# continental/uncertainty-detection-autolabeling

Measured on AMD Instinct MI355X. Metric: images*MC-samples/sec, EfficientDet-D0 MC-dropout serve (preprocess+net xT+decode+NMS), higher is better.
Workload: dtype f32 (tensors and accumulators float32; 1x1 products on the matrix cores as two fp16 pieces per operand, 3 cross terms (~2^-22 per product; float32-class, the default))

## Files before the change

uncertainty-detection-autolabeling_amd/csrc/kernels_pwb.hip:

```cpp
#include <math.h>
#include <stdio.h>
#include <stdlib.h>
#include <string.h>

#include <type_traits>

#include "mfma_common.h"

namespace uda {

template <int MT, int NT, int WM, int WN, int PARTS, int OCC, bool DEEP = false>
__global__ __launch_bounds__(256, OCC) void pwb_kernel(PwArgs a) {
  static_assert(WM * WN == 4, "four waves per block");
  constexpr int NPC = split_np(PARTS);
  constexpr int BM = 32 * MT * WM, NTB = NT * WN, BN = 32 * NTB;
  constexpr int A_BYTES = NPC * BM * PWB_AROW;
  constexpr int B_BYTES = 2 * NTB * NPC * 1024;
  constexpr int STG_BYTES = 4 * 32 * PWB_STG * 4;
  constexpr int LDS_BYTES = (A_BYTES + B_BYTES) > STG_BYTES ? (A_BYTES + B_BYTES) : STG_BYTES;
  __shared__ __attribute__((aligned(16))) unsigned char lds[LDS_BYTES];
  unsigned char* As = lds;
  uint4* Bs = (uint4*)(lds + A_BYTES);

  const int tid = threadIdx.x, lane = tid & 63, wave = tid >> 6;
// ... 265 lines not shown
#pragma unroll
    for (int p = 0; p < 2; ++p)
      bf[ks][p] = __builtin_bit_cast(bf16x8, ks < KS ? Wp[(((size_t)ks * NTL) * 2 + p) * 64 + lane] : make_uint4(0u, 0u, 0u, 0u));
  const int rrow = lane >> 4, c4 = lane & 15;
  const int col = 4 * c4;
  const bool colok = col < a.Cout;
  float4 bias = make_float4(0.f, 0.f, 0.f, 0.f), sc = make_float4(1.f, 1.f, 1.f, 1.f), sh = make_float4(0.f, 0.f, 0.f, 0.f);
  if (colok && (a.Cout & 3) == 0) {
    if (a.bias) bias = *(const float4*)(a.bias + col);
    if (a.bn_scale) { sc = *(const float4*)(a.bn_scale + col); sh = *(const float4*)(a.bn_shift + col); }
  }

  for (int t = 0; t < a.in_div; ++t) {
    const int b = b_in * a.in_div + t;
    float4 rg = make_float4(1.f, 1.f, 1.f, 1.f);
    if (a.se) {
      const int k = 4 * (lane & 7);
      if (k < a.Cin) rg = *(const float4*)(a.se + (size_t)(b / a.se_div) * a.Cin + k);
    }
#pragma unroll
    for (int i = 0; i < 4; ++i) {
      const int m = (lane >> 3) + 8 * i, kq = lane & 7;
      float r0 = ra[i].x * rg.x, r1 = ra[i].y * rg.y, r2 = ra[i].z * rg.z, r3 = ra[i].w * rg.w;
#pragma unroll
      for (int p = 0; p < 2; ++p) {
        const unsigned u0 = pack_bf16(r0, r1), u1 = pack_bf16(r2, r3);
        *(uint2*)(Aw + (size_t)(p * 32 + m) * PWB_AROW + kq * 8) = make_uint2(u0, u1);
        if (p == 0) {
          r0 -= bf16_lo_f32(u0); r1 -= bf16_hi_f32(u0);
          r2 -= bf16_lo_f32(u1); r3 -= bf16_hi_f32(u1);
        }
      }
    }
    __builtin_amdgcn_wave_barrier();
    f32x16 acc;
#pragma unroll
    for (int r = 0; r < 16; ++r) acc[r] = 0.f;
#pragma unroll
    for (int ks = 0; ks < 2; ++ks) {
      const bf16x8 a0 = *(const bf16x8*)(Aw + (size_t)(0 * 32 + li) * PWB_AROW + ks * 32 + lh * 16);
      const bf16x8 a1 = *(const bf16x8*)(Aw + (size_t)(1 * 32 + li) * PWB_AROW + ks * 32 + lh * 16);
      acc = __builtin_amdgcn_mfma_f32_32x32x16_bf16(a1, bf[ks][0], acc, 0, 0, 0);
      acc = __builtin_amdgcn_mfma_f32_32x32x16_bf16(a0, bf[ks][1], acc, 0, 0, 0);
      acc = __builtin_amdgcn_mfma_f32_32x32x16_bf16(a0, bf[ks][0], acc, 0, 0, 0);
    }
    __builtin_amdgcn_wave_barrier();
#pragma unroll
    for (int r = 0; r < 16; ++r) stg[((r & 3) + 8 * (r >> 2) + 4 * lh) * PWB_STG + li] = acc[r];
    __builtin_amdgcn_wave_barrier();
    float4 mk = make_float4(1.f, 1.f, 1.f, 1.f);
    if (colok && a.mask) mk = *(const float4*)(a.mask + (size_t)b * a.Cout + col);
    const size_t out_base = (size_t)b * a.HW;
    const size_t res_base = a.res ? (size_t)(b / a.res_div) * a.HW : 0;
#pragma unroll
    for (int it = 0; it < 8; ++it) {
      const int row = it * 4 + rrow;
      const int m = m0 + row;
      if (colok && m < a.HW) {
        float4 v = *(const float4*)(stg + row * PWB_STG + col);
        v.x = fmaf(v.x + bias.x, sc.x, sh.x);
        v.y = fmaf(v.y + bias.y, sc.y, sh.y);
        v.z = fmaf(v.z + bias.z, sc.z, sh.z);
        v.w = fmaf(v.w + bias.w, sc.w, sh.w);
        if (a.act == UDA_ACT_SWISH) {
          v.x = swishf_b(v.x); v.y = swishf_b(v.y); v.z = swishf_b(v.z); v.w = swishf_b(v.w);
        } else if (a.act >= UDA_ACT_RELU) {
          v.x = act_relu_family(v.x, a.act); v.y = act_relu_family(v.y, a.act); v.z = act_relu_family(v.z, a.act); v.w = act_relu_family(v.w, a.act);
        }
        v.x *= mk.x; v.y *= mk.y; v.z *= mk.z; v.w *= mk.w;
        if (a.res) {
          const float4 rr = *(const float4*)(a.res + (res_base + m) * a.Cout + col);
          v.x += rr.x; v.y += rr.y; v.z += rr.z; v.w += rr.w;
        }
        *(float4*)(a.out + (out_base + m) * a.Cout + col) = v;
      }
    }
    __builtin_amdgcn_wave_barrier();
  }
}

#ifndef UDA_PWS_D
#define UDA_PWS_D 4
#endif
constexpr int PWS_D = UDA_PWS_D;
template <int PARTS, int NT, bool GATE, bool IH = false>
__global__ __launch_bounds__(64) void pws_kernel(PwArgs a) {
  constexpr int NPC = split_np(PARTS);
  const int lane = threadIdx.x, li = lane & 31, lh = lane >> 5;
  const int m0 = blockIdx.x * 32, nt0 = blockIdx.y * NT;
  const int b = blockIdx.z, b_in = b / a.in_div;
  const int KS = a.Cin >> 4;
  const int NTL = (a.Cout + 31) >> 5;
  const int mr = m0 + li < a.HW ? m0 + li : a.HW - 1;
  const float* arow = a.in + ((size_t)b_in * a.HW + mr) * a.Cin + 8 * lh;
  constexpr bool in_h = IH;
  const unsigned short* arow_h = (const unsigned short*)a.in + ((size_t)b_in * a.HW + mr) * a.Cin + 8 * lh;
  const float* se = GATE ? a.se + (size_t)(b / a.se_div) * a.Cin + 8 * lh : nullptr;
  const uint4* Wp = (const uint4*)a.wsplit + lane;
  size_t woff[NT];
#pragma unroll
  for (int n = 0; n < NT; ++n) woff[n] = (size_t)(nt0 + n < NTL ? nt0 + n : NTL - 1) * NPC * 64;
  const size_t wks = (size_t)NTL * NPC * 64;

  f32x16 acc[NT];
#pragma unroll
  for (int n = 0; n < NT; ++n)
#pragma unroll
    for (int r = 0; r < 16; ++r) acc[n][r] = 0.f;
  float amax = 0.f;

  struct Step { float4 a0, a1, g0, g1; uint4 w[NT][NPC]; };
  struct Group { Step s[PWS_D]; };
  auto load_step = [&](int ks, Step& t) {
    if constexpr (in_h) {
      const uint4 h = *(const uint4*)(arow_h + 16 * ks);
      t.a0 = make_float4(__uint_as_float(h.x), __uint_as_float(h.y), __uint_as_float(h.z), __uint_as_float(h.w));
      t.a1 = t.a0;
    } else {
      t.a0 = *(const float4*)(arow + 16 * ks);
      t.a1 = *(const float4*)(arow + 16 * ks + 4);
    }
    if constexpr (GATE) {
      t.g0 = *(const float4*)(se + 16 * ks);
      t.g1 = *(const float4*)(se + 16 * ks + 4);
    }
#pragma unroll
    for (int n = 0; n < NT; ++n)
#pragma unroll
      for (int p = 0; p < NPC; ++p) t.w[n][p] = Wp[(size_t)ks * wks + woff[n] + p * 64];
  };
  auto mma_step = [&](const Step& t) {
    float4 v0 = t.a0, v1 = t.a1;
    if constexpr (in_h) {
      v0 = half4_to_float4<PARTS>(__float_as_uint(t.a0.x), __float_as_uint(t.a0.y));
      v1 = half4_to_float4<PARTS>(__float_as_uint(t.a0.z), __float_as_uint(t.a0.w));
    }
    if constexpr (GATE) {
      v0.x *= t.g0.x; v0.y *= t.g0.y; v0.z *= t.g0.z; v0.w *= t.g0.w;
      v1.x *= t.g1.x; v1.y *= t.g1.y; v1.z *= t.g1.z; v1.w *= t.g1.w;
    }
    bf16x8 af[NPC];
    split_parts<PARTS>(v0, v1, af, amax);
#pragma unroll
    for (int n = 0; n < NT; ++n) {
      bf16x8 bf[NPC];
#pragma unroll
      for (int p = 0; p < NPC; ++p) bf[p] = __builtin_bit_cast(bf16x8, t.w[n][p]);
      acc[n] = mfma_terms<PARTS>(af, bf, acc[n]);
    }
  };
  auto load_group = [&](int g, Group& G) {
#pragma unroll
    for (int d = 0; d < PWS_D; ++d) load_step(g * PWS_D + d, G.s[d]);
  };
  auto mma_group = [&](const Group& G) {
#pragma unroll
    for (int d = 0; d < PWS_D; ++d) mma_step(G.s[d]);
  };
  const int ng = KS / PWS_D;
  Group c0, c1;
  load_group(0, c0);
  load_group(ng > 1 ? 1 : 0, c1);
#pragma unroll 1
  for (int g = 0; g < ng; g += 2) {
    mma_group(c0);
    load_group(g + 2 < ng ? g + 2 : ng - 1, c0);
    if (g + 1 < ng) mma_group(c1);
    load_group(g + 3 < ng ? g + 3 : ng - 1, c1);
  }
#pragma unroll 1
  for (int ks = ng * PWS_D; ks < KS; ++ks) {
    Step t;
    load_step(ks, t);
    mma_step(t);
  }
  split_report<PARTS>(amax, a.oor);

  const size_t out_base = (size_t)b * a.HW;
  const float un = a.wunscale;
  const size_t res_base = a.res ? (size_t)(b / a.res_div) * a.HW : 0;
#pragma unroll
  for (int n = 0; n < NT; ++n) {
    const int col = (nt0 + n) * 32 + li;
    if (nt0 + n >= NTL || col >= a.Cout) continue;
    const float bias = a.bias ? a.bias[col] : 0.f;
    const float sc = a.bn_scale ? a.bn_scale[col] : 1.f;
    const float sh = a.bn_scale ? a.bn_shift[col] : 0.f;
    const float mk = a.mask ? a.mask[(size_t)b * a.Cout + col] : 1.f;
#pragma unroll
    for (int r = 0; r < 16; ++r) {
      const int m = m0 + (r & 3) + 8 * (r >> 2) + 4 * lh;
      if (m >= a.HW) continue;
      float v = fmaf(acc[n][r], un, bias);
      v = fmaf(v, sc, sh);
      if (a.act == UDA_ACT_SWISH) v = swishf_b(v);
      else if (a.act >= UDA_ACT_RELU) v = act_relu_family(v, a.act);
      v *= mk;
      if (a.res) v += a.res[(res_base + m) * a.Cout + col];
      a.out[(out_base + m) * a.Cout + col] = v;
    }
  }
}

static int launch_pws(const PwArgs& a, int rows, hipStream_t s) {
  static long long max_work = -1;
  if (max_work < 0) { const char* e = getenv("UDA_PW_SKINNY"); max_work = e ? atoll(e) : 60000; }
  if ((long long)rows * a.HW * ((a.Cout + 31) / 32) > max_work || a.Cin < 256 || (a.Cin & 15) || !a.wsplit || a.wparts == UDA_SPLIT_NONE) return 0;
  const int row_tiles = (a.HW + 31) / 32, NTL = (a.Cout + 31) / 32;
  const int nt = ((long long)row_tiles * rows * NTL <= 1024) ? 1 : 2;
  const dim3 grid(row_tiles, (NTL + nt - 1) / nt, rows), block(64);
  auto go = [&](auto k1, auto k2) { if (nt == 1) hipLaunchKernelGGL(k1, grid, block, 0, s, a); else hipLaunchKernelGGL(k2, grid, block, 0, s, a); };
  if (a.wparts == UDA_SPLIT_F16X2) { if (a.se) go(pws_kernel<4, 1, true>, pws_kernel<4, 2, true>); else go(pws_kernel<4, 1, false>, pws_kernel<4, 2, false>); }
  else if (a.wparts == UDA_SPLIT_F16X1 && a.in_f16) { if (a.se) go(pws_kernel<5, 1, true, true>, pws_kernel<5, 2, true, true>); else go(pws_kernel<5, 1, false, true>, pws_kernel<5, 2, false, true>); }
  else if (a.wparts == UDA_SPLIT_F16X1) { if (a.se) go(pws_kernel<5, 1, true>, pws_kernel<5, 2, true>); else go(pws_kernel<5, 1, false>, pws_kernel<5, 2, false>); }
  else if (a.wparts == UDA_SPLIT_BF16X1 && a.in_f16) { if (a.se) go(pws_kernel<6, 1, true, true>, pws_kernel<6, 2, true, true>); else go(pws_kernel<6, 1, false, true>, pws_kernel<6, 2, false, true>); }
  else if (a.wparts == UDA_SPLIT_BF16X1) { if (a.se) go(pws_kernel<6, 1, true>, pws_kernel<6, 2, true>); else go(pws_kernel<6, 1, false>, pws_kernel<6, 2, false>); }
  else if (a.wparts == UDA_SPLIT_BF16X3) { if (a.se) go(pws_kernel<3, 1, true>, pws_kernel<3, 2, true>); else go(pws_kernel<3, 1, false>, pws_kernel<3, 2, false>); }
  else if (a.wparts == UDA_SPLIT_BF16X2) { if (a.se) go(pws_kernel<2, 1, true>, pws_kernel<2, 2, true>); else go(pws_kernel<2, 1, false>, pws_kernel<2, 2, false>); }
  else return 0;
  return 1;
}

template <int MT, int NT, int WM, int WN>
static void launch_pwb_cfg(const PwArgs& a, int rows, hipStream_t s) {
  constexpr int BM = 32 * MT * WM, BN = 32 * NT * WN;
  const dim3 grid((a.HW + BM - 1) / BM, (a.Cout + BN - 1) / BN, rows), block(256);
  if (a.wparts == UDA_SPLIT_BF16X3) hipLaunchKernelGGL((pwb_kernel<MT, NT, WM, WN, 3, 2>), grid, block, 0, s, a);
  else if (a.wparts == UDA_SPLIT_F16X1) {
    hipLaunchKernelGGL((pwb_kernel<MT, NT, WM, WN, 5, (MT * NT > 5 ? 2 : 3)>), grid, block, 0, s, a);
  }
  else if (a.wparts == UDA_SPLIT_BF16X1) hipLaunchKernelGGL((pwb_kernel<MT, NT, WM, WN, 6, (MT * NT > 5 ? 2 : 3)>), grid, block, 0, s, a);
  else if (a.wparts == UDA_SPLIT_F16X2) {
    if constexpr (MT * NT > 4) {
      if (a.Cin >= 384 && a.Cin % PWB_BK == 0 && a.Cout % BN == 0 && (2 * NT * WN * 2 * 64) % 256 == 0) { hipLaunchKernelGGL((pwb_kernel<MT, NT, WM, WN, 4, 2, true>), grid, block, 0, s, a); return; }
    }
    hipLaunchKernelGGL((pwb_kernel<MT, NT, WM, WN, 4, (MT * NT > 4 ? 2 : 3)>), grid, block, 0, s, a);
  }
  else hipLaunchKernelGGL((pwb_kernel<MT, NT, WM, WN, 2, (MT * NT > 4 ? 2 : 3)>), grid, block, 0, s, a);
}

void launch_pwb(const PwArgs& a, int rows, hipStream_t s) {
  static const int shared = uda_env_int("UDA_PW_SHARED", 1);
  if (shared && a.in_div > 1 && a.Cin <= 32 && a.Cout <= 32 && (a.Cout & 3) == 0 && a.wparts == 2 && rows % a.in_div == 0) {
    const dim3 grid((a.HW + 127) / 128, 1, rows / a.in_div);
    hipLaunchKernelGGL(pwb_shared_kernel, grid, dim3(256), 0, s, a);
    return;
  }
  if (launch_pws(a, rows, s)) return;
  int cfg = a.Cout <= 32 ? 1 : (a.Cout <= 64 ? 2 : (a.Cout <= 96 ? 3 : 4));
  if (a.Cout > 128) {
    const int bn[3] = {128, 160, 192}, id[3] = {4, 6, 5};
    int best = 1 << 30;
    for (int i = 0; i < 3; ++i) {
      const int waste = (a.Cout + bn[i] - 1) / bn[i] * bn[i] - a.Cout;
      if (waste <= best) { best = waste; cfg = id[i]; }
    }
  }
  switch (cfg) {
    case 1: launch_pwb_cfg<1, 1, 4, 1>(a, rows, s); break;
    case 2: launch_pwb_cfg<1, 2, 4, 1>(a, rows, s); break;
    case 3: launch_pwb_cfg<1, 3, 4, 1>(a, rows, s); break;
    case 5: launch_pwb_cfg<2, 3, 2, 2>(a, rows, s); break;
    case 6: launch_pwb_cfg<1, 5, 4, 1>(a, rows, s); break;
    default: launch_pwb_cfg<2, 2, 2, 2>(a, rows, s); break;
  }
}

#ifndef UDA_MBX_ET
#define UDA_MBX_ET 3
#endif
__host__ __device__ constexpr int mbx_et_w(int k, int s) {
  return s != 1 ? 0 : (k == 5 ? ((UDA_MBX_ET & 1) ? 4 : 0) : ((UDA_MBX_ET & 2) ? 2 : 0));
}
__host__ __device__ constexpr int mbx_et_pitch(int w) { return w == 2 ? 258 : 260; }
template <int W>
__device__ __forceinline__ void et_store_slice(float* ep, const f32x16& acc) {
#pragma unroll
  for (int q = 0; q < 4; ++q) {
    const float v0 = swish_core(acc[4 * q]), v1 = swish_core(acc[4 * q + 1]), v2 = swish_core(acc[4 * q + 2]), v3 = swish_core(acc[4 * q + 3]);
    if constexpr (W == 4) {
      *(float4*)(ep + 8 * q) = make_float4(v0, v1, v2, v3);
    } else {
      *(float2*)(ep + 8 * q) = make_float2(v0, v1);
      *(float2*)(ep + 8 * q + 2) = make_float2(v2, v3);
    }
  }
}
template <int W>
__device__ __forceinline__ void et_read(float* dst, const float* er, int jj) {
  if constexpr (W == 4) {
    const float4 v = *(const float4*)(er + 4 * jj);
    dst[4 * jj] = v.x; dst[4 * jj + 1] = v.y; dst[4 * jj + 2] = v.z; dst[4 * jj + 3] = v.w;
  } else {
    const float2 v = *(const float2*)(er + 2 * jj);
    dst[2 * jj] = v.x; dst[2 * jj + 1] = v.y;
  }
}

namespace {
struct MbxCfgB { int th, tw; };
__host__ __device__ constexpr MbxCfgB mbxb_cfg(int k, int s) {
  return s == 1 ? (k == 3 ? MbxCfgB{12, 16} : MbxCfgB{8, 16}) : (k == 3 ? MbxCfgB{7, 8} : MbxCfgB{4, 10});
}
}

#ifndef UDA_MBXB_WK_LDS
#define UDA_MBXB_WK_LDS 1
#endif
#ifndef UDA_MBXB6_W
#define UDA_MBXB6_W 3
#endif
#ifndef UDA_MBXB_MINW
#define UDA_MBXB_MINW(K, S, KSF, PARTS) ((PARTS) == 3 ? (((KSF) <= 2 && (K) == 3) ? UDA_MBXB6_W : 2) : \
    ((KSF) <= 2 ? ((K) == 3 ? 4 : 3) : (((KSF) <= 3 && ((K) == 3 ? (S) == 2 : UDA_MBXB_WK_LDS)) ? 3 : 2)))
#endif
template <int K, int S, int KSF, bool FUSE0, int PARTS, bool OH = false>
__global__ __launch_bounds__(256, UDA_MBXB_MINW(K, S, KSF, PARTS)) void mbxb_kernel(MbxArgs a) {
  constexpr int NW = 4;
  constexpr int NPC = split_np(PARTS);
  constexpr int TH = mbxb_cfg(K, S).th, TW = mbxb_cfg(K, S).tw;
  constexpr int IH = (TH - 1) * S + K, IW = (TW - 1) * S + K;
  constexpr int NP = IH * IW;
  constexpr int NPP = (NP + 31) / 32 * 32;
  constexpr int NMT = NPP / 32;
  constexpr int NG = NW * 2;
  constexpr int MTW = (NMT + NW - 1) / NW;
  constexpr int ES = 32;
  constexpr int ETW = mbx_et_w(K, S);
  constexpr bool ET = ETW != 0;
  constexpr int CP = mbx_et_pitch(ETW);
  constexpr int XW = (S == 1) ? 8 : (K == 3 ? (TW == 8 ? 8 : 6) : 5);
  constexpr int UPR = TW / XW;
  constexpr int NUNIT = TH * UPR;
  static_assert(TW % XW == 0, "units must tile the output tile");
  constexpr int NCOL = (XW - 1) * S + K;
  extern __shared__ __attribute__((aligned(16))) float mlds[];
  float* E = mlds;
  float* red = E + (ET ? (size_t)32 * CP : (size_t)NPP * ES);
  constexpr int NPAR = (K * K + 2) * 32;
  float* par = red + NG * 32;
  constexpr bool B_LDS = KSF <= 2;
  constexpr int BSLAB = KSF * NPC * 64;
  uint4* Bs = (uint4*)(par + 2 * NPAR);

  const int tid = threadIdx.x, lane = tid & 63, wave = tid >> 6;
  const int li = lane & 31, lh = lane >> 5;
  int tbx = blockIdx.x, tby = blockIdx.y, b = blockIdx.z;
  if (a.remap_T > 0) {
    const int T = a.remap_T, nt = a.tiles_x * a.tiles_y, ntp = (nt + 7) & ~7;
    const unsigned L = blockIdx.x;
    const unsigned per_img = (unsigned)ntp * (unsigned)T;
    const int img = (int)(L / per_img);
    const unsigned r = L - (unsigned)img * per_img;
    const int grp = (int)(r / (8u * (unsigned)T)), w = (int)(r % (8u * (unsigned)T));
    const int tl = grp * 8 + (w & 7);
    if (tl >= nt) return;
    b = img * T + (w >> 3);
    tby = tl / a.tiles_x;
    tbx = tl - tby * a.tiles_x;
  }
  const int b_in = b / a.in_div;
  const int oy0 = tby * TH, ox0 = tbx * TW;
  const int iy0 = oy0 * S - a.pad_t, ix0 = ox0 * S - a.pad_l;
  const int cin_mem = FUSE0 ? a.c0 : a.Cin;
  const float* xin = a.in + (size_t)b_in * a.H * a.W * cin_mem;

  float amax = 0.f;
  bf16x8 w0p[2][NPC];
  float sh0v[8];
  if constexpr (FUSE0) {
    if (a.w0frag) {
      const uint4* fp = a.w0frag + (size_t)(b / a.g_div) * (2 * NPC * 64) + lane;
#pragma unroll
      for (int ks = 0; ks < 2; ++ks)
#pragma unroll
        for (int p_ = 0; p_ < NPC; ++p_) w0p[ks][p_] = __builtin_bit_cast(bf16x8, fp[(ks * NPC + p_) * 64]);
    } else {
      const float* gp = a.gate + (size_t)(b / a.g_div) * a.c0;
#pragma unroll
      for (int ks = 0; ks < 2; ++ks) {
        const int k = ks * 16 + 8 * lh;
        float4 w0 = *(const float4*)(a.w0t + li * 32 + k), w1 = *(const float4*)(a.w0t + li * 32 + k + 4);
        const float4 g0 = *(const float4*)(gp + k), g1 = *(const float4*)(gp + k + 4);
        w0.x *= g0.x; w0.y *= g0.y; w0.z *= g0.z; w0.w *= g0.w;
        w1.x *= g1.x; w1.y *= g1.y; w1.z *= g1.z; w1.w *= g1.w;
        split_parts<PARTS>(w0, w1, w0p[ks], amax);
      }
    }
#pragma unroll
    for (int j = 0; j < 8; ++j) sh0v[j] = a.sh0f[(j & 3) + 8 * (j >> 2) + 4 * lh];
  }

  bf16x8 ap[MTW][KSF][NPC];
#pragma unroll
  for (int t = 0; t < MTW; ++t) {
    const int mt = wave + NW * t;
    const int p = mt * 32 + li;
    const int iy = iy0 + p / IW, ix = ix0 + p % IW;
    const bool in = (mt < NMT) && (p < NP) && iy >= 0 && iy < a.H && ix >= 0 && ix < a.W;
    const float* px = xin + ((size_t)(in ? iy : 0) * a.W + (in ? ix : 0)) * cin_mem;
    if constexpr (FUSE0) {
      static_assert(!FUSE0 || KSF == 2, "the fused projection feeds a 16-channel expand");
      f32x16 xacc;
#pragma unroll
      for (int r = 0; r < 16; ++r) xacc[r] = 0.f;
#pragma unroll
      for (int ks = 0; ks < 2; ++ks) {
        const int k = ks * 16 + 8 * lh;
        float4 d0 = make_float4(0.f, 0.f, 0.f, 0.f), d1 = d0;
        if (in) {
          d0 = *(const float4*)(px + k);
          d1 = *(const float4*)(px + k + 4);
        }
        bf16x8 dp[NPC];
        split_parts<PARTS>(d0, d1, dp, amax);
        xacc = mfma_terms<PARTS>(w0p[ks], dp, xacc);
      }
      float4 v0, v1;
      v0.x = in ? xacc[0] + sh0v[0] : 0.f; v0.y = in ? xacc[1] + sh0v[1] : 0.f;
      v0.z = in ? xacc[2] + sh0v[2] : 0.f; v0.w = in ? xacc[3] + sh0v[3] : 0.f;
      v1.x = in ? xacc[4] + sh0v[4] : 0.f; v1.y = in ? xacc[5] + sh0v[5] : 0.f;
      v1.z = in ? xacc[6] + sh0v[6] : 0.f; v1.w = in ? xacc[7] + sh0v[7] : 0.f;
      split_parts<PARTS>(v0, v1, ap[t][0], amax);
      float4 f0 = make_float4((lh == 0 && in) ? 1.f : 0.f, 0.f, 0.f, 0.f), f1 = make_float4(0.f, 0.f, 0.f, 0.f);
      split_parts<PARTS>(f0, f1, ap[t][1]);
      continue;
    }
#pragma unroll
    for (int ks = 0; ks < KSF; ++ks) {
      const int k = ks * 16 + 8 * lh;
      float4 v0 = make_float4(0.f, 0.f, 0.f, 0.f), v1 = v0;
      if (in && k < a.Cin) {
        v0 = *(const float4*)(px + k);
        v1 = *(const float4*)(px + k + 4);
      }
      if (k == a.Cin) v0.x = in ? 1.f : 0.f;
      split_parts<PARTS>(v0, v1, ap[t][ks], amax);
    }
  }
  split_report<PARTS>(amax, a.oor);

  const int c = tid & 31, g = tid >> 5;
  const size_t tile = (size_t)tby * ((a.Wo + TW - 1) / TW) + tbx;
  const int NCH = (a.Cmid + 31) >> 5;
  const uint4* Wp = (const uint4*)a.wsplit;

  constexpr int UPT = (NUNIT + NG - 1) / NG;
  constexpr bool UNIT_GUARD = (NUNIT % NG) != 0;
  int eoff[UPT];
  unsigned ooff[UPT];
#pragma unroll
  for (int ui = 0; ui < UPT; ++ui) {
    const int u = (UNIT_GUARD && g + NG * ui >= NUNIT) ? 0 : g + NG * ui;
    const int orow = u / UPR, oxs = (u % UPR) * XW;
    eoff[ui] = ET ? c * CP + (orow * S) * IW + oxs * S : ((orow * S) * IW + oxs * S) * ES + c;
    ooff[ui] = (unsigned)((orow * a.Wo + oxs) * a.Cmid + c) * 4u;
  }
  float* const obase = a.out + (((size_t)b * a.Ho + oy0) * a.Wo + ox0) * a.Cmid;
  const unsigned cm = (unsigned)a.Cmid;
  unsigned short* const hobase = (unsigned short*)a.out + (((size_t)b * a.Ho + oy0) * a.Wo + ox0) * a.Cmid;
  const bool full = (oy0 + TH <= a.Ho) && (ox0 + TW <= a.Wo);

  constexpr int P_PER = (NPAR + 255) / 256;
  constexpr int B_PER = (BSLAB + 255) / 256;
  auto b_src = [&](int ch, int f) -> const uint4* {
    const int ks = f / (NPC * 64), rest = f - ks * (NPC * 64);
    return Wp + (((size_t)ks * NCH + ch) * NPC + (rest >> 6)) * 64 + (rest & 63);
  };
  constexpr int KR = B_LDS ? 1 : KSF;
  uint4 rb[KR][NPC], nbr[KR][NPC];
  auto load_regs = [&](int ch, uint4 (*dst)[NPC]) {
#pragma unroll
    for (int ks = 0; ks < KR; ++ks)
#pragma unroll
      for (int p_ = 0; p_ < NPC; ++p_) dst[ks][p_] = Wp[(((size_t)ks * NCH + ch) * NPC + p_) * 64 + lane];
  };
  if constexpr (B_LDS) {
    for (int f = tid; f < BSLAB; f += 256) Bs[f] = *b_src(0, f);
  } else {
    load_regs(0, rb);
  }
  for (int f = tid; f < NPAR; f += 256) par[f] = a.wpar[f];
  auto mask_at = [&](const float* m, int ch) -> float {
    const int col_ = ch * 32 + c;
    const float* mp = m ? m + (size_t)b * a.Cmid + (col_ < a.Cmid ? col_ : 0) : a.wpar;
    const float v = *mp;
    return (m ? v : 1.f) * UDA_NEG_LN2;
  };
  float mk0 = mask_at(a.mask0, 0), mk0n = mk0;
  float mk1 = mask_at(a.mask1, 0), mk1n = mk1;
  __syncthreads();

  for (int ch = 0; ch < NCH; ++ch) {
    const int col = ch * 32 + c;
    const bool dcol = col < a.Cmid;
    const float* pcur = par + (ch & 1) * NPAR;
    const bool more = ch + 1 < NCH;
    const int chn = more ? ch + 1 : ch;
    uint4 nb[B_PER];
    if constexpr (B_LDS) {
#pragma unroll
      for (int i = 0; i < B_PER; ++i) {
        const int f = tid + 256 * i;
        nb[i] = *b_src(chn, f < BSLAB ? f : 0);
      }
    } else {
      load_regs(chn, nbr);
    }
    float np_[P_PER];
    const float* wnext = a.wpar + (size_t)chn * NPAR;
#pragma unroll
    for (int i = 0; i < P_PER; ++i) {
      const int f = tid + 256 * i;
      np_[i] = wnext[f < NPAR ? f : 0];
    }
    mk0n = mask_at(a.mask0, chn);
    mk1n = mask_at(a.mask1, chn);
    bf16x8 bp[KSF][NPC];
#pragma unroll
    for (int ks = 0; ks < KSF; ++ks)
#pragma unroll
      for (int p_ = 0; p_ < NPC; ++p_) {
        if constexpr (B_LDS) bp[ks][p_] = __builtin_bit_cast(bf16x8, Bs[(ks * NPC + p_) * 64 + lane]);
        else bp[ks][p_] = __builtin_bit_cast(bf16x8, rb[ks < KR ? ks : 0][p_]);
      }
#pragma unroll
    for (int t = 0; t < MTW; ++t) {
      const int mt = wave + NW * t;
      if (mt < NMT) {
        f32x16 acc;
#pragma unroll
        for (int r = 0; r < 16; ++r) acc[r] = 0.f;
#pragma unroll
        for (int ks = 0; ks < KSF; ++ks) acc = mfma_terms<PARTS>(ap[t][ks], bp[ks], acc);
        if constexpr (ET) {
          et_store_slice<ETW>(E + li * CP + mt * 32 + 4 * lh, acc);
        } else {
          float* ep = E + (size_t)(mt * 32 + 4 * lh) * ES + li;
#pragma unroll
          for (int r = 0; r < 16; ++r) ep[((r & 3) + 8 * (r >> 2)) * ES] = swish_core(acc[r]);
        }
      }
    }
    __syncthreads();
    {
      if constexpr (B_LDS) {
#pragma unroll
        for (int i = 0; i < B_PER; ++i) {
          const int f = tid + 256 * i;
          if (more && f < BSLAB) Bs[f] = nb[i];
        }
      } else {
#pragma unroll
        for (int ks = 0; ks < KR; ++ks)
#pragma unroll
          for (int p_ = 0; p_ < NPC; ++p_)
            asm volatile("" : "+v"(nbr[ks][p_].x), "+v"(nbr[ks][p_].y), "+v"(nbr[ks][p_].z), "+v"(nbr[ks][p_].w));
      }
      float* pnext = par + ((ch + 1) & 1) * NPAR;
#pragma unroll
      for (int i = 0; i < P_PER; ++i) {
        const int f = tid + 256 * i;
        if (more && f < NPAR) pnext[f] = np_[i];
      }
      asm volatile("" : "+v"(mk0n), "+v"(mk1n));
    }
    constexpr bool WK_LDS = UDA_MBXB_WK_LDS && K == 5 && KSF == 3;
    float wk[WK_LDS ? 1 : K * K];
    if constexpr (!WK_LDS) {
#pragma unroll
      for (int t = 0; t < K * K; ++t) wk[t] = pcur[t * 32 + c];
    }
    const float sc1 = pcur[K * K * 32 + c] * mk0, sh1 = pcur[(K * K + 1) * 32 + c];
    float ssum = 0.f;
    float* const ob = obase + ch * 32;
    unsigned short* const hob = hobase + ch * 32;
    auto dw_units = [&](auto guard) {
      constexpr bool GUARD = decltype(guard)::value;
      constexpr int KYU = (UDA_MBXB_WK_LDS && K == 5 && KSF == 3) ? 1 : K;
#pragma unroll
      for (int ui = 0; ui < UPT; ++ui) {
        if constexpr (UNIT_GUARD) {
          if (g + NG * ui >= NUNIT) continue;
        }
        if constexpr (GUARD) {
          if (oy0 + (g + NG * ui) / UPR >= a.Ho) continue;
        }
        float acc[XW];
#pragma unroll
        for (int o = 0; o < XW; ++o) acc[o] = 0.f;
        const float* eu = E + eoff[ui];
#pragma unroll KYU
        for (int ky = 0; ky < K; ++ky) {
          float rowv[NCOL];
          if constexpr (ET) {
            static_assert(!ET || NCOL % ETW == 0, "whole 16- / 8-byte reads");
#pragma unroll
            for (int jj = 0; jj < NCOL / (ET ? ETW : 1); ++jj) et_read<ETW>(rowv, eu + ky * IW, jj);
          } else {
#pragma unroll
            for (int j = 0; j < NCOL; ++j) rowv[j] = eu[(ky * IW + j) * ES];
          }
#pragma unroll
          for (int kx = 0; kx < K; ++kx) {
            const float w = WK_LDS ? pcur[(ky * K + kx) * 32 + c] : wk[WK_LDS ? 0 : ky * K + kx];
#pragma unroll
            for (int o = 0; o < XW; ++o) acc[o] = fmaf(rowv[o * S + kx], w, acc[o]);
          }
        }
#pragma unroll
        for (int o = 0; o < XW; ++o) {
          bool ok = true;
          if constexpr (GUARD) ok = ox0 + (int)((g + NG * ui) % UPR) * XW + o < a.Wo;
          if (ok) {
            const float v = swish_folded(fmaf(acc[o], sc1, sh1), mk1);
            if constexpr (OH) store_uniform_base_16<PARTS>(hob + (size_t)o * cm, ooff[ui], v);
            else store_uniform_base(ob + (size_t)o * cm, ooff[ui], v);
            ssum += v;
          }
        }
        __builtin_amdgcn_sched_barrier(0);
      }
    };
    if (dcol) {
      if (full) dw_units(std::false_type());
      else dw_units(std::true_type());
    }
    if (a.se_partial) red[g * 32 + c] = ssum;
    __syncthreads();
    if (a.se_partial && g == 0 && dcol) {
      float t = red[c];
#pragma unroll
      for (int gg = 1; gg < NG; ++gg) t += red[gg * 32 + c];
      a.se_partial[((size_t)b * a.n_tiles + tile) * a.Cmid + col] = t;
    }
    mk0 = mk0n;
    mk1 = mk1n;
    if constexpr (!B_LDS) {
#pragma unroll
      for (int ks = 0; ks < KR; ++ks)
#pragma unroll
        for (int p_ = 0; p_ < NPC; ++p_) rb[ks][p_] = nbr[ks][p_];
    }
  }
}

template <int PARTS>
__global__ __launch_bounds__(64) void w0gate_kernel(const float* gate, const float* w0t, int c0, uint4* out, unsigned* oor) {
  constexpr int NPC = split_np(PARTS);
  const int row = blockIdx.x, lane = threadIdx.x, li = lane & 31, lh = lane >> 5;
  const float* gp = gate + (size_t)row * c0;
  float amax = 0.f;
#pragma unroll
  for (int ks = 0; ks < 2; ++ks) {
    const int k = ks * 16 + 8 * lh;
    float4 w0 = *(const float4*)(w0t + li * 32 + k), w1 = *(const float4*)(w0t + li * 32 + k + 4);
    const float4 g0 = *(const float4*)(gp + k), g1 = *(const float4*)(gp + k + 4);
    w0.x *= g0.x; w0.y *= g0.y; w0.z *= g0.z; w0.w *= g0.w;
    w1.x *= g1.x; w1.y *= g1.y; w1.z *= g1.z; w1.w *= g1.w;
    bf16x8 pc[NPC];
    split_parts<PARTS>(w0, w1, pc, amax);
#pragma unroll
    for (int p_ = 0; p_ < NPC; ++p_) out[((size_t)row * 2 * NPC + ks * NPC + p_) * 64 + lane] = __builtin_bit_cast(uint4, pc[p_]);
  }
  split_report<PARTS>(amax, oor);
}

size_t mbxb_w0frag_elems(int gate_rows, int scheme) { return (size_t)gate_rows * 2 * uda_split_pieces(scheme) * 64; }
void launch_w0gate(const float* gate, const float* w0t, int c0, int gate_rows, int scheme, uint4* out, unsigned* oor, hipStream_t s) {
  if (scheme == UDA_SPLIT_BF16X3) hipLaunchKernelGGL(w0gate_kernel<3>, dim3(gate_rows), dim3(64), 0, s, gate, w0t, c0, out, oor);
  else if (scheme == UDA_SPLIT_F16X2) hipLaunchKernelGGL(w0gate_kernel<4>, dim3(gate_rows), dim3(64), 0, s, gate, w0t, c0, out, oor);
  else if (scheme == UDA_SPLIT_F16X1) hipLaunchKernelGGL(w0gate_kernel<5>, dim3(gate_rows), dim3(64), 0, s, gate, w0t, c0, out, oor);
  else if (scheme == UDA_SPLIT_BF16X1) hipLaunchKernelGGL(w0gate_kernel<6>, dim3(gate_rows), dim3(64), 0, s, gate, w0t, c0, out, oor);
  else hipLaunchKernelGGL(w0gate_kernel<2>, dim3(gate_rows), dim3(64), 0, s, gate, w0t, c0, out, oor);
}

int mbxb_tiles(int Ho, int Wo, int k, int stride) {
  const MbxCfgB c = mbxb_cfg(k, stride);
  return ((Ho + c.th - 1) / c.th) * ((Wo + c.tw - 1) / c.tw);
}

bool mbxb_supported(int Cin, int Cmid, int k, int stride) {
  return Cin % 8 == 0 && Cin >= 16 && Cin <= 48 && Cmid % 4 == 0 && (k == 3 || k == 5) && (stride == 1 || stride == 2);
}

template <int K, int S, int KSF, int PARTS>
static void launch_mbxb_t(const MbxArgs& a, int rows, hipStream_t s) {
  constexpr int TH = mbxb_cfg(K, S).th, TW = mbxb_cfg(K, S).tw;
  constexpr int IH = (TH - 1) * S + K, IW = (TW - 1) * S + K;
  constexpr int NPP = (IH * IW + 31) / 32 * 32;
  const size_t lds = ((mbx_et_w(K, S) ? (size_t)32 * mbx_et_pitch(mbx_et_w(K, S)) : (size_t)NPP * 32) + 8 * 32 + 2 * (K * K + 2) * 32) * sizeof(float) +
                     (size_t)KSF * split_np(PARTS) * 64 * sizeof(uint4);
  dim3 grid((a.Wo + TW - 1) / TW, (a.Ho + TH - 1) / TH, rows);
  MbxArgs b = a;
  b.remap_T = 0;
  if (a.in_div > 1 && rows % a.in_div == 0) {
    const long long nt = (long long)grid.x * grid.y, ntp = (nt + 7) / 8 * 8;
    const long long total = ntp * rows;
    if (total < (1ll << 31)) {
      b.remap_T = a.in_div; b.tiles_x = (int)grid.x; b.tiles_y = (int)grid.y;
      grid = dim3((unsigned)total, 1, 1);
    }
  }
  if constexpr (split_one(PARTS)) {
    if (a.out_f16) {
      if constexpr (KSF == 2) {
        if (a.gate) { hipLaunchKernelGGL((mbxb_kernel<K, S, KSF, true, PARTS, true>), grid, dim3(256), lds, s, b); return; }
      }
      hipLaunchKernelGGL((mbxb_kernel<K, S, KSF, false, PARTS, true>), grid, dim3(256), lds, s, b);
      return;
    }
  }
  if constexpr (KSF == 2) {
    if (a.gate) { hipLaunchKernelGGL((mbxb_kernel<K, S, KSF, true, PARTS>), grid, dim3(256), lds, s, b); return; }
  }
  hipLaunchKernelGGL((mbxb_kernel<K, S, KSF, false, PARTS>), grid, dim3(256), lds, s, b);
}

template <int K, int S, int PARTS>
static void launch_mbxb_ks(const MbxArgs& a, int rows, hipStream_t s) {
  switch ((a.Cin + 1 + 15) / 16) {
    case 2: launch_mbxb_t<K, S, 2, PARTS>(a, rows, s); break;
    case 3: launch_mbxb_t<K, S, 3, PARTS>(a, rows, s); break;
    default: launch_mbxb_t<K, S, 4, PARTS>(a, rows, s); break;
  }
}

template <int PARTS>
static void launch_mbxb_p(const MbxArgs& a, int rows, int k, int stride, hipStream_t s) {
  if (k == 3 && stride == 1) launch_mbxb_ks<3, 1, PARTS>(a, rows, s);
  else if (k == 3 && stride == 2) launch_mbxb_ks<3, 2, PARTS>(a, rows, s);
  else if (k == 5 && stride == 1) launch_mbxb_ks<5, 1, PARTS>(a, rows, s);
  else launch_mbxb_ks<5, 2, PARTS>(a, rows, s);
}

void launch_mbxb(const MbxArgs& a, int rows, int k, int stride, hipStream_t s) {
  if (a.wparts == UDA_SPLIT_BF16X3) launch_mbxb_p<3>(a, rows, k, stride, s);
  else if (a.wparts == UDA_SPLIT_F16X2) launch_mbxb_p<4>(a, rows, k, stride, s);
  else if (a.wparts == UDA_SPLIT_F16X1) launch_mbxb_p<5>(a, rows, k, stride, s);
  else if (a.wparts == UDA_SPLIT_BF16X1) launch_mbxb_p<6>(a, rows, k, stride, s);
  else launch_mbxb_p<2>(a, rows, k, stride, s);
}

struct MbxCfgD { int th, tw, xw; };
__host__ __device__ constexpr MbxCfgD mbxd_cfg(int k, int s, bool wide = false) {
  return s == 1 ? (wide ? (k == 3 ? MbxCfgD{8, 20, 10} : MbxCfgD{6, 20, 4}) : (k == 3 ? MbxCfgD{12, 16, 4} : MbxCfgD{8, 16, 8}))
                : (k == 3 ? MbxCfgD{7, 8, 8} : MbxCfgD{4, 10, 5});
}
__host__ __device__ constexpr long long mbxd_slots(int Ho, int Wo, int k, bool wide) {
  return (long long)((Ho + mbxd_cfg(k, 1, wide).th - 1) / mbxd_cfg(k, 1, wide).th) * mbxd_cfg(k, 1, wide).th *
         ((Wo + mbxd_cfg(k, 1, wide).tw - 1) / mbxd_cfg(k, 1, wide).tw) * mbxd_cfg(k, 1, wide).tw;
}
bool mbxd_wide(int Ho, int Wo, int k, int stride) {
  return stride == 1 && mbxd_slots(Ho, Wo, k, true) < mbxd_slots(Ho, Wo, k, false);
}

__host__ __device__ constexpr bool mbxd_two_per_cu(int ksf, int parts, int s) { return (ksf <= 8 && parts != 3) || (split_one(parts) && s == 1); }
template <int K, int KSF, int PARTS, int S, bool WIDE, bool OH = false>
__global__ __launch_bounds__(512, mbxd_two_per_cu(KSF, PARTS, S) ? 4 : 2) void mbxd_kernel(MbxArgs a) {
  constexpr bool WK_LDS = (K == 5 && (KSF <= 8 || PARTS == 3 || split_one(PARTS)));

  constexpr int NW = 8;
  constexpr int NPC = split_np(PARTS);
  static_assert(!WIDE || S == 1, "wide tiles are a stride-1 variant");
  constexpr int TH = mbxd_cfg(K, S, WIDE).th, TW = mbxd_cfg(K, S, WIDE).tw;
  constexpr int IH = (TH - 1) * S + K, IW = (TW - 1) * S + K;
  constexpr int NP = IH * IW;
  static_assert(NP <= 256, "input tile must fit 8 slices of 32 pixels");
  constexpr int NPP = 256;
  constexpr int NG = NW * 2;
  constexpr int ES = 33;
  constexpr int ETW = mbx_et_w(K, S);
  constexpr bool ET = ETW != 0;
  constexpr int CP = mbx_et_pitch(ETW);
  static_assert(!ET || (IW % ETW == 0 && mbxd_cfg(K, S, WIDE).xw % ETW == 0), "aligned wide accesses of the transposed slab");
  constexpr int XW = mbxd_cfg(K, S, WIDE).xw;
  constexpr int UPR = TW / XW;
  constexpr int NUNIT = TH * UPR;
  static_assert(TW % XW == 0, "units must tile the output tile");
  constexpr int NCOL = (XW - 1) * S + K;
  constexpr int BSLAB = KSF * NPC * 64;
  extern __shared__ __attribute__((aligned(16))) float dlds[];
  float* E = dlds;
  float* red = E + (size_t)NPP * ES;
  constexpr int NPAR = (K * K + 2) * 32;
  float* par = red + NG * 32;
  uint4* Bs = (uint4*)(par + 2 * NPAR);
  float* mks = (float*)(Bs + BSLAB);

  const int tid = threadIdx.x, lane = tid & 63, wave = tid >> 6;
  const int li = lane & 31, lh = lane >> 5;
  const int b = blockIdx.z / a.ch_groups, b_in = b / a.in_div;
  const int oy0 = blockIdx.y * TH, ox0 = blockIdx.x * TW;
  const int iy0 = oy0 * S - a.pad_t, ix0 = ox0 * S - a.pad_l;
  const float* xin = a.in + (size_t)b_in * a.H * a.W * a.Cin;
  const int NCH = (a.Cmid + 31) >> 5;
  const int ch_per = (NCH + a.ch_groups - 1) / a.ch_groups;
  const int chb = (int)(blockIdx.z % a.ch_groups) * ch_per;
  const int che = chb + ch_per < NCH ? chb + ch_per : NCH;
  if (chb >= che) return;
  const uint4* Wp = (const uint4*)a.wsplit;
  for (int f = tid; f < BSLAB; f += 512) {
    const int ks = f / (NPC * 64), rest = f - ks * (NPC * 64);
    Bs[f] = Wp[(((size_t)ks * NCH + chb) * NPC + (rest >> 6)) * 64 + (rest & 63)];
  }
  for (int f = tid; f < NPAR; f += 512) par[f] = a.wpar[(size_t)chb * NPAR + f];
  for (int f = tid; f < 2 * 32 * NCH; f += 512) {
    const int which = f / (32 * NCH), col = f - which * 32 * NCH;
    const float* m = which ? a.mask1 : a.mask0;
    mks[f] = ((m && col < a.Cmid) ? m[(size_t)b * a.Cmid + col] : 1.f) * UDA_NEG_LN2;
  }

  bf16x8 ap[KSF][NPC];
  float amax = 0.f;
  {
    const int p = wave * 32 + li;
    const int iy = iy0 + p / IW, ix = ix0 + p % IW;
    const bool in = (p < NP) && iy >= 0 && iy < a.H && ix >= 0 && ix < a.W;
    const float* px = xin + ((size_t)(in ? iy : 0) * a.W + (in ? ix : 0)) * a.Cin;
#pragma unroll
    for (int ks = 0; ks < KSF; ++ks) {
      const int k = ks * 16 + 8 * lh;
      float4 v0 = make_float4(0.f, 0.f, 0.f, 0.f), v1 = v0;
      if (in && k < a.Cin) {
        v0 = *(const float4*)(px + k);
        v1 = *(const float4*)(px + k + 4);
      }
      if (k == a.Cin) v0.x = in ? 1.f : 0.f;
      split_parts<PARTS>(v0, v1, ap[ks], amax);
    }
  }
  split_report<PARTS>(amax, a.oor);
  __syncthreads();

  const int c = tid & 31, g = tid >> 5;
  const size_t tile = (size_t)blockIdx.y * gridDim.x + blockIdx.x;
  constexpr int B_PER = (BSLAB + 511) / 512;
  constexpr int UPT = (NUNIT + NG - 1) / NG;
  constexpr bool UNIT_GUARD = (NUNIT % NG) != 0;
  int eoff[UPT];
  unsigned ooff[UPT];
#pragma unroll
  for (int ui = 0; ui < UPT; ++ui) {
    const int u = (UNIT_GUARD && g + NG * ui >= NUNIT) ? 0 : g + NG * ui;
    const int orow = u / UPR, oxs = (u % UPR) * XW;
    eoff[ui] = ET ? c * CP + orow * S * IW + oxs * S : (orow * S * IW + oxs * S) * ES + c;
    ooff[ui] = (unsigned)((orow * a.Wo + oxs) * a.Cmid + c) * 4u;
  }
  float* const obase = a.out + (((size_t)b * a.Ho + oy0) * a.Wo + ox0) * a.Cmid;
  const unsigned cm = (unsigned)a.Cmid;
  unsigned short* const hobase = (unsigned short*)a.out + (((size_t)b * a.Ho + oy0) * a.Wo + ox0) * a.Cmid;
  const bool full = (oy0 + TH <= a.Ho) && (ox0 + TW <= a.Wo);

  for (int ch = chb; ch < che; ++ch) {
    const int col = ch * 32 + c;
    const bool dcol = col < a.Cmid;
    const uint4* bcur = Bs;
    const float mk0c = mks[ch * 32 + c], mk1 = mks[32 * NCH + ch * 32 + c];
    const float* pcur = par + ((ch - chb) & 1) * NPAR;
    const bool more = ch + 1 < che;
    uint4 nb[B_PER];
#pragma unroll
    for (int i = 0; i < B_PER; ++i) {
      const int f = tid + 512 * i;
      const int ks = f / (NPC * 64), rest = f - ks * (NPC * 64);
      uint4 v = make_uint4(0u, 0u, 0u, 0u);
      if (more && f < BSLAB) v = Wp[(((size_t)ks * NCH + (ch + 1)) * NPC + (rest >> 6)) * 64 + (rest & 63)];
      nb[i] = v;
    }
    constexpr int P_PER = (NPAR + 511) / 512;
    float np_[P_PER];
    const float* wnext = a.wpar + (size_t)(more ? ch + 1 : ch) * NPAR;
#pragma unroll
    for (int i = 0; i < P_PER; ++i) {
      const int f = tid + 512 * i;
      np_[i] = wnext[f < NPAR ? f : 0];
    }
    {
      f32x16 acc;
#pragma unroll
      for (int r = 0; r < 16; ++r) acc[r] = 0.f;
#pragma unroll
      for (int ks = 0; ks < KSF; ++ks) {
        bf16x8 bp[NPC];
#pragma unroll
        for (int p_ = 0; p_ < NPC; ++p_) bp[p_] = __builtin_bit_cast(bf16x8, bcur[(ks * NPC + p_) * 64 + lane]);
        acc = mfma_terms<PARTS>(ap[ks], bp, acc);
      }
      if constexpr (ET) {
        et_store_slice<ETW>(E + li * CP + wave * 32 + 4 * lh, acc);
      } else {
        float* ep = E + (size_t)(wave * 32 + 4 * lh) * ES + li;
#pragma unroll
        for (int r = 0; r < 16; ++r) ep[((r & 3) + 8 * (r >> 2)) * ES] = swish_core(acc[r]);
      }
    }
    __syncthreads();
    {
#pragma unroll
      for (int i = 0; i < B_PER; ++i) {
        const int f = tid + 512 * i;
        if (more && f < BSLAB) Bs[f] = nb[i];
      }
      float* pnext = par + ((ch + 1 - chb) & 1) * NPAR;
#pragma unroll
      for (int i = 0; i < P_PER; ++i) {
        const int f = tid + 512 * i;
        if (more && f < NPAR) pnext[f] = np_[i];
      }
    }
    float wk[WK_LDS ? 1 : K * K];
    if constexpr (!WK_LDS) {
#pragma unroll
      for (int t = 0; t < K * K; ++t) wk[t] = pcur[t * 32 + c];
    }
    const float sc1 = pcur[K * K * 32 + c] * mk0c, sh1 = pcur[(K * K + 1) * 32 + c];
    float ssum = 0.f;
    float* const ob = obase + ch * 32;
    unsigned short* const hob = hobase + ch * 32;
    auto dw_units = [&](auto guard) {
      constexpr bool GUARD = decltype(guard)::value;
#pragma unroll
      for (int ui = 0; ui < UPT; ++ui) {
        if constexpr (UNIT_GUARD) {
          if (g + NG * ui >= NUNIT) continue;
        }
        if constexpr (GUARD) {
          if (oy0 + (g + NG * ui) / UPR >= a.Ho) continue;
        }
        float acc[XW];
#pragma unroll
        for (int o = 0; o < XW; ++o) acc[o] = 0.f;
        const float* eu = E + eoff[ui];
        constexpr int KYU = WK_LDS ? 1 : K;
#pragma unroll KYU
        for (int ky = 0; ky < K; ++ky) {
          float rowv[NCOL];
          if constexpr (ET) {
            static_assert(!ET || NCOL % ETW == 0, "whole 16- / 8-byte reads");
#pragma unroll
            for (int jj = 0; jj < NCOL / (ET ? ETW : 1); ++jj) et_read<ETW>(rowv, eu + ky * IW, jj);
          } else {
            const float* er = eu + ky * IW * ES;
#pragma unroll
            for (int j = 0; j < NCOL; ++j) rowv[j] = er[j * ES];
// ... 648 lines not shown
```

Measured before the change: 5296.

## Add half-width tail path for depthwise expand when channel count ends in 16

When Cmid mod 32 is 16, the final 32-channel chunk of the fused expand+depthwise kernel is now handled by a dedicated tail path. It computes only the live 16 columns and spreads 256 threads as 16 channels by 16 groups with a retuned unit width per kernel/stride. The aim is to stop wasting half the depthwise lanes and stores on padded channels in the last chunk. This adds a second code path with new LDS layout constraints and higher register and code-size pressure.

Result: no change. 5327 (median of 6 runs) (+0.6%).

```diff
diff --git a/uncertainty-detection-autolabeling_amd/csrc/kernels_pwb.hip b/uncertainty-detection-autolabeling_amd/csrc/kernels_pwb.hip
--- a/uncertainty-detection-autolabeling_amd/csrc/kernels_pwb.hip
+++ b/uncertainty-detection-autolabeling_amd/csrc/kernels_pwb.hip
@@ -591,6 +591,11 @@
 __host__ __device__ constexpr MbxCfgB mbxb_cfg(int k, int s) {
   return s == 1 ? (k == 3 ? MbxCfgB{12, 16} : MbxCfgB{8, 16}) : (k == 3 ? MbxCfgB{7, 8} : MbxCfgB{4, 10});
 }
+struct MbxTailCfg { int xw, upr; };
+__host__ __device__ constexpr MbxTailCfg mbxb_tail_cfg(int k, int s) {
+  return s == 1 ? (k == 3 ? MbxTailCfg{4, 4} : MbxTailCfg{8, 2}) : (k == 3 ? MbxTailCfg{4, 2} : MbxTailCfg{3, 4});
+}
+constexpr int MBX_TAIL_EP = 20;
 }
 
 #ifndef UDA_MBXB_WK_LDS
@@ -780,7 +785,10 @@
   float mk1 = mask_at(a.mask1, 0), mk1n = mk1;
   __syncthreads();
 
-  for (int ch = 0; ch < NCH; ++ch) {
+  constexpr bool TAIL = NPC == 2 && !FUSE0 && !OH && !(K == 3 && S == 2 && KSF == 3);
+  const bool tail = TAIL && (a.Cmid & 31) == 16;
+  const int NFULL = tail ? NCH - 1 : NCH;
+  for (int ch = 0; ch < NFULL; ++ch) {
     const int col = ch * 32 + c;
     const bool dcol = col < a.Cmid;
     const float* pcur = par + (ch & 1) * NPAR;
@@ -930,6 +938,144 @@
       for (int ks = 0; ks < KR; ++ks)
 #pragma unroll
         for (int p_ = 0; p_ < NPC; ++p_) rb[ks][p_] = nbr[ks][p_];
+    }
+  }
+
+  if constexpr (TAIL) {
+    if (tail) {
+      constexpr int NGT = 16;
+      constexpr int TXW = mbxb_tail_cfg(K, S).xw, TUPR = mbxb_tail_cfg(K, S).upr;
+      constexpr bool RAGGED = TXW * TUPR != TW;
+      static_assert(RAGGED ? (TXW == 3 && TUPR == 4 && TW == 10) : true, "ragged cut: 3 + 3 + 2 + 2");
+      constexpr int TNUNIT = TH * TUPR;
+      constexpr int TUPT = (TNUNIT + NGT - 1) / NGT;
+      constexpr bool TUNIT_GUARD = (TNUNIT % NGT) != 0;
+      constexpr int TNCOL = (TXW - 1) * S + K;
+      constexpr int TEP = MBX_TAIL_EP;
+      static_assert(ET || (size_t)NPP * TEP <= (size_t)NPP * ES, "the tail slab lives inside E");
+      static_assert(!RAGGED || ((TH - 1) * S + K - 1) * IW + 8 * S + TNCOL - 1 < NPP, "ragged window stays inside the slab");
+      const int ch = NCH - 1;
+      int ttid = tid;
+      asm volatile("" : "+v"(ttid));
+      const int tc = ttid & 15, tg = ttid >> 4;
+      const int tli = ttid & 31, tlh = (ttid >> 5) & 1, twave = ttid >> 6;
+      const int tcol = ch * 32 + tc;
+      const float* pcur = par + (ch & 1) * NPAR;
+      const float tm0 = (a.mask0 ? a.mask0[(size_t)b * a.Cmid + tcol] : 1.f) * UDA_NEG_LN2;
+      const float tm1 = (a.mask1 ? a.mask1[(size_t)b * a.Cmid + tcol] : 1.f) * UDA_NEG_LN2;
+      bf16x8 bp[KSF][NPC];
+#pragma unroll
+      for (int ks = 0; ks < KSF; ++ks)
+#pragma unroll
+        for (int p_ = 0; p_ < NPC; ++p_) {
+          if constexpr (B_LDS) bp[ks][p_] = __builtin_bit_cast(bf16x8, Bs[(ks * NPC + p_) * 64 + lane]);
+          else bp[ks][p_] = __builtin_bit_cast(bf16x8, rb[ks < KR ? ks : 0][p_]);
+        }
+#pragma unroll
+      for (int t = 0; t < MTW; ++t) {
+        const int mt = wave + NW * t;
+        if (mt < NMT) {
+          f32x16 acc;
+#pragma unroll
+          for (int r = 0; r < 16; ++r) acc[r] = 0.f;
+#pragma unroll
+          for (int ks = 0; ks < KSF; ++ks) {
+            acc = mfma16<PARTS>(bp[ks][0], ap[t][ks][1], acc);
+            acc = mfma16<PARTS>(bp[ks][1], ap[t][ks][0], acc);
+            acc = mfma16<PARTS>(bp[ks][0], ap[t][ks][0], acc);
+          }
+          const int tp = (twave + NW * t) * 32 + tli;
+          if constexpr (ET) {
+            float* ep = E + (4 * tlh) * CP + tp;
+#pragma unroll
+            for (int r = 0; r < 8; ++r) ep[((r & 3) + 8 * (r >> 2)) * CP] = swish_core(acc[r]);
+          } else {
+            float* ep = E + tp * TEP + 4 * tlh;
+            *(float4*)ep = make_float4(swish_core(acc[0]), swish_core(acc[1]), swish_core(acc[2]), swish_core(acc[3]));
+            *(float4*)(ep + 8) = make_float4(swish_core(acc[4]), swish_core(acc[5]), swish_core(acc[6]), swish_core(acc[7]));
+          }
+        }
+      }
+      __syncthreads();
+      int teoff[TUPT];
+      unsigned tooff[TUPT];
+#pragma unroll
+      for (int ui = 0; ui < TUPT; ++ui) {
+        const int u = (TUNIT_GUARD && tg + NGT * ui >= TNUNIT) ? 0 : tg + NGT * ui;
+        const int orow = u / TUPR, q = u % TUPR;
+        const int oxs = RAGGED ? q * TXW - (q == 3 ? 1 : 0) : q * TXW;
+        teoff[ui] = ET ? tc * CP + (orow * S) * IW + oxs * S : ((orow * S) * IW + oxs * S) * TEP + tc;
+        tooff[ui] = (unsigned)((orow * a.Wo + oxs) * a.Cmid + tc) * 4u;
+      }
+      constexpr bool WK_LDS = UDA_MBXB_WK_LDS && K == 5 && KSF == 3;
+      float wk[WK_LDS ? 1 : K * K];
+      if constexpr (!WK_LDS) {
+#pragma unroll
+        for (int t = 0; t < K * K; ++t) wk[t] = pcur[t * 32 + tc];
+      }
+      const float sc1 = pcur[K * K * 32 + tc] * tm0, sh1 = pcur[(K * K + 1) * 32 + tc];
+      float ssum = 0.f;
+      float* const ob = obase + ch * 32;
+      auto dw_tail = [&](auto guard) {
+        constexpr bool GUARD = decltype(guard)::value;
+        constexpr int KYU = WK_LDS ? 1 : K;
+#pragma unroll
+        for (int ui = 0; ui < TUPT; ++ui) {
+          const int u = tg + NGT * ui;
+          if constexpr (TUNIT_GUARD) {
+            if (u >= TNUNIT) continue;
+          }
+          if constexpr (GUARD) {
+            if (oy0 + u / TUPR >= a.Ho) continue;
+          }
+          const int q = u % TUPR;
+          float acc[TXW];
+#pragma unroll
+          for (int o = 0; o < TXW; ++o) acc[o] = 0.f;
+          const float* eu = E + teoff[ui];
+#pragma unroll KYU
+          for (int ky = 0; ky < K; ++ky) {
+            float rowv[TNCOL];
+            if constexpr (ET) {
+              static_assert(!ET || TNCOL % ETW == 0, "whole 16- / 8-byte reads");
+#pragma unroll
+              for (int jj = 0; jj < TNCOL / (ET ? ETW : 1); ++jj) et_read<ETW>(rowv, eu + ky * IW, jj);
+            } else {
+#pragma unroll
+              for (int j = 0; j < TNCOL; ++j) rowv[j] = eu[(ky * IW + j) * TEP];
+            }
+#pragma unroll
+            for (int kx = 0; kx < K; ++kx) {
+              const float w = WK_LDS ? pcur[(ky * K + kx) * 32 + tc] : wk[WK_LDS ? 0 : ky * K + kx];
+#pragma unroll
+              for (int o = 0; o < TXW; ++o) acc[o] = fmaf(rowv[o * S + kx], w, acc[o]);
+            }
+          }
+          const int oxs = RAGGED ? q * TXW - (q == 3 ? 1 : 0) : q * TXW;
+#pragma unroll
+          for (int o = 0; o < TXW; ++o) {
+            bool ok = true;
+            if constexpr (RAGGED) ok = o < 2 || q < 2;
+            if constexpr (GUARD) ok = ok && ox0 + oxs + o < a.Wo;
+            if (ok) {
+              const float v = swish_folded(fmaf(acc[o], sc1, sh1), tm1);
+              store_uniform_base(ob + (size_t)o * cm, tooff[ui], v);
+              ssum += v;
+            }
+          }
+          __builtin_amdgcn_sched_barrier(0);
+        }
+      };
+      if (full) dw_tail(std::false_type());
+      else dw_tail(std::true_type());
+      if (a.se_partial) red[tg * 16 + tc] = ssum;
+      __syncthreads();
+      if (a.se_partial && tg == 0) {
+        float t = red[tc];
+#pragma unroll
+        for (int gg = 1; gg < NGT; ++gg) t += red[gg * 16 + tc];
+        a.se_partial[((size_t)b * a.n_tiles + tile) * a.Cmid + tcol] = t;
+      }
     }
   }
 }
```
